# microsoft/tf-gnn-samples

Measured on AMD Instinct MI355X. Metric: edges/sec (whole node), RGCN PPI h=256 training, distinct batches (the reference's epoch-loop definition), higher is better.
Workload: dtype f32; 1 GPU; C2: RGCN on synthetic PPI-shaped batches (~16 graphs, ~1.88 M edges, ~32 k nodes each), 3 edge types [fwd,self,bkwd], h=256, 3 layers, sum aggregation, 1/in-de…; graphs_per_rank=64, max_nodes_in_batch=35964, input_pipeline=ResidentDataset, parallelism=dp1-by-graph

## Files before the change

tf_gnn_samples_amd/_lib.py:

```python
import ctypes
from pathlib import Path

import torch

_PKG_DIR = Path(__file__).resolve().parent
LIB_PATH = _PKG_DIR / "librelgnn.so"

OK, EINVAL, ENOSPC, EHIP, EUNSUPPORTED = 0, 1, 2, 3, 4
ERRFLAG_INDEX_OUT_OF_RANGE = 1
ERRFLAG_NOT_SORTED = 2

AGG_SUM, AGG_MEAN, AGG_SQRT_N, AGG_MAX = 0, 1, 2, 3
MT_MAX = 48
ACT_LINEAR, ACT_TANH, ACT_RELU, ACT_LEAKY_RELU, ACT_ELU, ACT_SELU, ACT_GELU = range(7)

_c_i32, _c_i64, _c_f32 = ctypes.c_int32, ctypes.c_int64, ctypes.c_float
_c_u32 = ctypes.c_uint32
_ptr = ctypes.c_void_p

ABI = {}

ABI["relgnn.h"] = {
    "relgnn_abi_version": (ctypes.c_int, []),
    "relgnn_status_string": (ctypes.c_char_p, [ctypes.c_int]),
# ... 216 lines not shown

ABI["relgnn_sparse_gradient.h"] = {
    "relgnn_named_rows_workspace_bytes": (ctypes.c_size_t, [_c_i64]),
    "relgnn_named_rows_count": (ctypes.c_int, [_ptr, _c_i64, _ptr, _ptr, _ptr, ctypes.c_size_t, _ptr]),
    "relgnn_named_rows_fill": (ctypes.c_int, [_ptr, _c_i64, _ptr, _c_i64, _ptr, _ptr, _ptr, _ptr, _c_i64, _ptr, _ptr, _c_i64, _ptr]),
    "relgnn_rows_l2norm_workspace_bytes": (ctypes.c_size_t, []),
    "relgnn_rows_l2norm": (ctypes.c_int, [_ptr, _c_i64, _ptr, _c_i64, _c_i32, _c_i64, _ptr, _ptr, ctypes.c_size_t, _ptr]),
    "relgnn_rows_adam_step_compact": (ctypes.c_int, [_ptr, _c_i64, _c_i64, _ptr, _ptr, _c_i64, _ptr, _ptr, _c_i64, _c_i32, _ptr, _ptr, _c_i32,
                                                     _c_i32, _ptr, _c_f32, _c_f32, _c_f32, _c_f32, _c_f32, _ptr]),
}

ABI["relgnn_subgraph.h"] = {
    "relgnn_subgraph_supported": (ctypes.c_int, [_c_i64, _c_i32, _c_i64, _c_i32]),
    "relgnn_subgraph_max_walk_length": (_c_i64, []),
    "relgnn_subgraph_workspace_bytes": (ctypes.c_size_t, [_c_i64]),
    "relgnn_subgraph_walk": (ctypes.c_int, [_ptr, _ptr, _c_i64, _c_i32, _ptr, _c_i64, _c_i32, _c_u32, _c_u32, _c_u32, _ptr, _ptr]),
    "relgnn_subgraph_number": (ctypes.c_int, [_ptr, _ptr, _c_i64, _ptr, _c_i64, _ptr]),
    "relgnn_subgraph_induced_count": (ctypes.c_int, [_ptr, _ptr, _c_i64, _c_i32, _ptr, _ptr, _c_i64, _ptr, _ptr, _ptr, _ptr, _ptr,
                                                     ctypes.c_size_t, _ptr]),
    "relgnn_subgraph_induced_emit": (ctypes.c_int, [_ptr, _ptr, _c_i64, _c_i32, _ptr, _c_i64, _c_i64, _ptr, _ptr, _c_i64, _ptr, _ptr,
                                                    _ptr]),
    "relgnn_subgraph_clear": (ctypes.c_int, [_ptr, _c_i64, _ptr, _c_i64, _ptr]),
}

ABI["relgnn_subgraph_norm.h"] = {
    "relgnn_subgraph_visit_count": (ctypes.c_int, [_ptr, _ptr, _c_i64, _c_i32, _c_i64, _ptr, _ptr, _c_i64, _ptr, _ptr, _ptr, _ptr]),
    "relgnn_subgraph_induced_emit_weighted": (ctypes.c_int, [_ptr, _ptr, _c_i64, _c_i32, _c_i64, _ptr, _c_i64, _c_i64, _ptr, _ptr, _ptr,
                                                             _ptr, _c_f32, _c_i64, _ptr, _ptr, _ptr, _ptr]),
    "relgnn_softmax_ce_weighted_stats_workspace_bytes": (ctypes.c_size_t, []),
    "relgnn_softmax_ce_weighted_stats": (ctypes.c_int, [_ptr, _c_i64, _ptr, _ptr, _ptr, _c_f32, _c_i64, _c_i32, _ptr, _ptr,
                                                        ctypes.c_size_t, _ptr]),
    "relgnn_softmax_ce_weighted_bwd": (ctypes.c_int, [_ptr, _c_i64, _ptr, _ptr, _ptr, _c_f32, _c_i64, _c_i32, _ptr, _ptr, _ptr, _c_i64,
                                                      _ptr]),
}

INTERNAL = {}

INTERNAL["graph_partition.h"] = {
    "relgnn_partition_supported": (ctypes.c_int, [_c_i64, _c_i32, _c_i64, _c_i32, _c_i32]),
    "relgnn_partition_wave_row_max": (_c_i64, []),
    "relgnn_partition_wish": (ctypes.c_int, [_ptr, _ptr, _c_i64, _c_i32, _c_i64, _ptr, _ptr, _c_i32, _ptr, _c_i32, _c_u32, _c_u32, _ptr, _ptr,
                                             _c_i64, _c_i32, _ptr, _ptr]),
}

INTERNAL["level_plan.h"] = {
    "relgnn_level_plan_max_levels": (_c_i32, []),
    "relgnn_level_plan_desc_stride": (_c_i64, [_c_i32]),
    "relgnn_level_plan_tile": (_c_i64, []),
    "relgnn_level_plan_workspace_bytes": (ctypes.c_size_t, [_c_i64, _c_i32]),
    "relgnn_level_plan": (ctypes.c_int, [_ptr, _ptr, _ptr, _ptr, _ptr, _ptr, _ptr, _ptr, _ptr, _c_i64, _c_i32, _c_i64, _ptr, _c_i32, _c_i64,
                                         _c_i64, _ptr, _c_i64, _ptr, ctypes.c_size_t, _ptr]),
}

_lib = None


class RelGnnLibraryError(RuntimeError):
    pass


def load_library():
    global _lib
    if _lib is not None:
        return _lib
    if not LIB_PATH.exists():
        raise RelGnnLibraryError(
            "%s not found: the HIP extension is not built. Run `python -c 'import __graft_entry__ as g; "
            "g.build()'` (needs hipcc). There is no CPU fallback for this path." % LIB_PATH)
    lib = ctypes.CDLL(str(LIB_PATH))
    typed = signatures()
    for header, table in INTERNAL.items():
        for name in table:
            if name in typed:
                raise RelGnnLibraryError("%s of csrc/%s is bound twice" % (name, header))
        typed.update(table)
    for name, (restype, argtypes) in typed.items():
        fn = getattr(lib, name)
        fn.restype = restype
        fn.argtypes = argtypes
    if lib.relgnn_abi_version() != 1:
        raise RelGnnLibraryError("librelgnn.so ABI version mismatch")
    _lib = lib
    return lib


def signatures(header=None):
    if header is not None:
        return dict(ABI[header])
    union, owner = {}, {}
    for h, table in ABI.items():
        for name in table:
            if name in owner:
                raise RelGnnLibraryError("%s is bound by both %s and %s" % (name, owner[name], h))
            owner[name] = h
        union.update(table)
    return union


def status_string(code: int) -> str:
    return load_library().relgnn_status_string(code).decode()


def check(code: int, what: str):
    if code == OK:
        return
    msg = "%s failed: %s (status %d)" % (what, status_string(code), code)
# ... 34 lines not shown
```

tf_gnn_samples_amd/csrc/plan_resident.hip:

```cpp
#include "common.h"

using namespace relgnn;

namespace {

__device__ __forceinline__ int upper_slot(const int64_t* __restrict__ table, int n, int64_t x) {
  int lo = 0, hi = n;
  while (hi - lo > 1) {
    const int mid = (lo + hi) >> 1;
    if (table[mid] <= x) lo = mid; else hi = mid;
  }
  return lo;
}

struct BatchTables {
  const int64_t* ids;
  const int64_t* node_off_b;
  const int64_t* msg_off_b;
  const int64_t* edge_off_b;
  const int64_t* type_off_b;
  const int64_t* node_off_d;
  const int64_t* msg_off_d;
  const int64_t* edge_off_d;
  const int64_t* type_off_d;
  int32_t K, L;
  int64_t G;
};

__device__ __forceinline__ int32_t translate_message(const BatchTables& t, int32_t m_d, int l, int k, int64_t g) {
  const int64_t e = (int64_t)m_d - t.type_off_d[l] - t.edge_off_d[(int64_t)l * (t.G + 1) + g];
  return (int32_t)(t.type_off_b[l] + t.edge_off_b[(int64_t)l * (t.K + 1) + k] + e);
}

template <bool FULL>
__global__ __launch_bounds__(256) void assemble_by_target_kernel(
    BatchTables t, int64_t M, const int32_t* __restrict__ perm_d, const int32_t* __restrict__ col_d,
    int32_t* __restrict__ perm_b, int32_t* __restrict__ col_b, int32_t* __restrict__ inv_b,
    const float* __restrict__ w_t_d, int32_t* __restrict__ src_b, float* __restrict__ w_t_b) {
  __shared__ int first_slot;
  for (int64_t base = (int64_t)blockIdx.x * 1024; base < M; base += (int64_t)gridDim.x * 1024) {
    if (threadIdx.x == 0) first_slot = upper_slot(t.msg_off_b, t.K, base);
    __syncthreads();
    int k = first_slot;
    int64_t g = t.ids[k], slot_end = t.msg_off_b[k + 1];
    int64_t msg_delta = t.msg_off_d[g] - t.msg_off_b[k], node_delta = t.node_off_b[k] - t.node_off_d[g];
#pragma unroll
    for (int e = 0; e < 4; ++e) {
      const int64_t p = base + threadIdx.x + 256 * e;
      if (p >= M) break;
      if (p >= slot_end) {
        do { ++k; } while (p >= t.msg_off_b[k + 1]);
        g = t.ids[k]; slot_end = t.msg_off_b[k + 1];
        msg_delta = t.msg_off_d[g] - t.msg_off_b[k]; node_delta = t.node_off_b[k] - t.node_off_d[g];
      }
      const int64_t pd = p + msg_delta;
      const uint32_t c = (uint32_t)col_d[pd];
      const uint32_t cn = c / (uint32_t)t.L;
      const int64_t src = (int64_t)cn + node_delta;
      if (src_b) src_b[p] = (int32_t)src;
      if (w_t_b) w_t_b[p] = w_t_d[pd];
      if constexpr (FULL) {
        const int l = (int)(c - cn * (uint32_t)t.L);
        col_b[p] = (int32_t)(src * t.L + l);
        const int32_t mb = translate_message(t, perm_d[pd], l, k, g);
        perm_b[p] = mb;
        inv_b[mb] = (int32_t)p;
      }
    }
    __syncthreads();
  }
}

template <bool FULL>
__global__ __launch_bounds__(256) void assemble_by_source_kernel(
    BatchTables t, int64_t M, const int32_t* __restrict__ perm_d, const int32_t* __restrict__ frow_d,
    const int32_t* __restrict__ pos_d, int32_t* __restrict__ perm_b, int32_t* __restrict__ frow_b,
    int32_t* __restrict__ tgt_b, int32_t* __restrict__ pos_b, const float* __restrict__ w_s_d, float* __restrict__ w_s_b) {
  __shared__ int first_slot;
  for (int64_t base = (int64_t)blockIdx.x * 1024; base < M; base += (int64_t)gridDim.x * 1024) {
    if (threadIdx.x == 0) first_slot = upper_slot(t.msg_off_b, t.K, base);
    __syncthreads();
    int k = first_slot;
    int64_t g = t.ids[k], slot_end = t.msg_off_b[k + 1];
    int64_t msg_delta = t.msg_off_d[g] - t.msg_off_b[k], node_delta = t.node_off_b[k] - t.node_off_d[g];
#pragma unroll
    for (int e = 0; e < 4; ++e) {
      const int64_t q = base + threadIdx.x + 256 * e;
      if (q >= M) break;
      if (q >= slot_end) {
        do { ++k; } while (q >= t.msg_off_b[k + 1]);
        g = t.ids[k]; slot_end = t.msg_off_b[k + 1];
        msg_delta = t.msg_off_d[g] - t.msg_off_b[k]; node_delta = t.node_off_b[k] - t.node_off_d[g];
      }
      const int64_t qd = q + msg_delta;
      const uint32_t f = (uint32_t)frow_d[qd];
      const uint32_t fn = f / (uint32_t)t.L;
      const int64_t tgt = (int64_t)fn + node_delta;
      tgt_b[q] = (int32_t)tgt;
      if (w_s_b) w_s_b[q] = w_s_d[qd];
      if constexpr (FULL) {
        const int l = (int)(f - fn * (uint32_t)t.L);
        frow_b[q] = (int32_t)(tgt * t.L + l);
        perm_b[q] = translate_message(t, perm_d[qd], l, k, g);
        pos_b[q] = (int32_t)((int64_t)pos_d[qd] - msg_delta);
      }
    }
    __syncthreads();
  }
}

__global__ __launch_bounds__(256) void assemble_rowptr_kernel(
    BatchTables t, int64_t num_buckets, int64_t M, const int32_t* __restrict__ rowptr_t_d,
    const int32_t* __restrict__ rowptr_s_d, int32_t* __restrict__ rowptr_t_b, int32_t* __restrict__ rowptr_s_b) {
  for (int64_t b = blockIdx.x * (int64_t)blockDim.x + threadIdx.x; b <= num_buckets; b += (int64_t)gridDim.x * blockDim.x) {
    if (b == num_buckets) {
      rowptr_t_b[b] = (int32_t)M;
      rowptr_s_b[b] = (int32_t)M;
      continue;
    }
    const int64_t v = b / t.L;
    const int l = (int)(b - v * t.L);
    const int k = upper_slot(t.node_off_b, t.K, v);
    const int64_t g = t.ids[k];
    const int64_t bd = (v - t.node_off_b[k] + t.node_off_d[g]) * t.L + l;
    const int64_t shift = t.msg_off_b[k] - t.msg_off_d[g];
    rowptr_t_b[b] = (int32_t)((int64_t)rowptr_t_d[bd] + shift);
    rowptr_s_b[b] = (int32_t)((int64_t)rowptr_s_d[bd] + shift);
  }
}


__global__ __launch_bounds__(256) void gather_node_rows_kernel(BatchTables t, int64_t V, int32_t cols,
                                                               const uint32_t* __restrict__ src, uint32_t* __restrict__ dst) {
  __shared__ int first_slot;
  const int64_t total = V * cols;
  for (int64_t base = (int64_t)blockIdx.x * 1024; base < total; base += (int64_t)gridDim.x * 1024) {
    if (threadIdx.x == 0) {
      int lo = 0, hi = t.K;
      while (hi - lo > 1) {
        const int mid = (lo + hi) >> 1;
        if (t.node_off_b[mid] * cols <= base) lo = mid; else hi = mid;
      }
      first_slot = lo;
    }
    __syncthreads();
    int k = first_slot;
    int64_t slot_end = t.node_off_b[k + 1] * cols;
    int64_t delta = (t.node_off_d[t.ids[k]] - t.node_off_b[k]) * cols;
#pragma unroll
    for (int e = 0; e < 4; ++e) {
      const int64_t i = base + threadIdx.x + 256 * e;
      if (i < total) {
        if (i >= slot_end) {
          do { ++k; } while (i >= t.node_off_b[k + 1] * cols);
          slot_end = t.node_off_b[k + 1] * cols;
          delta = (t.node_off_d[t.ids[k]] - t.node_off_b[k]) * cols;
        }
        dst[i] = src[delta + i];
      }
    }
    __syncthreads();
  }
}

__global__ __launch_bounds__(256) void gather_degree_kernel(BatchTables t, int64_t V, int64_t N, const float* __restrict__ deg_d,
                                                            float* __restrict__ deg_b, int32_t* __restrict__ node_to_graph) {
  for (int64_t v = blockIdx.x * (int64_t)blockDim.x + threadIdx.x; v < V; v += (int64_t)gridDim.x * blockDim.x) {
    const int k = upper_slot(t.node_off_b, t.K, v);
    const int64_t vd = v - t.node_off_b[k] + t.node_off_d[t.ids[k]];
    for (int l = 0; l < t.L; ++l) deg_b[(int64_t)l * V + v] = deg_d[(int64_t)l * N + vd];
    node_to_graph[v] = k;
  }
}

__global__ __launch_bounds__(256) void gather_adjacency_kernel(BatchTables t, int64_t M, const int2* __restrict__ adj_d,
                                                               int2* __restrict__ adj_b) {
  for (int64_t p = blockIdx.x * (int64_t)blockDim.x + threadIdx.x; p < M; p += (int64_t)gridDim.x * blockDim.x) {
    const int l = upper_slot(t.type_off_b, t.L, p);
    const int64_t e = p - t.type_off_b[l];
    const int64_t* eob = t.edge_off_b + (int64_t)l * (t.K + 1);
    const int k = upper_slot(eob, t.K, e);
    const int64_t g = t.ids[k];
    const int64_t pd = t.type_off_d[l] + t.edge_off_d[(int64_t)l * (t.G + 1) + g] + (e - eob[k]);
    int2 a = adj_d[pd];
    const int off = (int)t.node_off_b[k];
    a.x += off; a.y += off;
    adj_b[p] = a;
  }
}

}

extern "C" {

int relgnn_batch_gather(const int64_t* ids, int32_t num_batch_graphs, int32_t num_edge_types, int64_t num_dataset_graphs,
                        const int64_t* node_off_b, const int64_t* edge_off_b, const int64_t* type_off_b,
                        const int64_t* node_off_d, const int64_t* edge_off_d, const int64_t* type_off_d, int64_t num_nodes,
                        int64_t num_messages, int64_t num_dataset_nodes, int32_t n_payloads, const void* const* h_payload_d,
                        const int32_t* h_payload_cols, void* const* h_payload_b, const float* deg_d, float* deg_b,
                        const int32_t* adj_d, int32_t* adj_b, int32_t* node_to_graph, void* stream) {
  if (num_batch_graphs < 0 || num_edge_types <= 0 || num_dataset_graphs < 0 || num_nodes < 0 || num_messages < 0 ||
      n_payloads < 0 || num_dataset_nodes < 0)
    return RELGNN_EINVAL;
  if (num_batch_graphs == 0 || num_nodes == 0) return RELGNN_OK;
  if (!ids || !node_off_b || !edge_off_b || !type_off_b || !node_off_d || !edge_off_d || !type_off_d) return RELGNN_EINVAL;
  if (n_payloads > 0 && (!h_payload_d || !h_payload_cols || !h_payload_b)) return RELGNN_EINVAL;
  hipStream_t st = as_stream(stream);
  BatchTables t{ids, node_off_b, nullptr, edge_off_b, type_off_b, node_off_d, nullptr, edge_off_d, type_off_d,
                num_batch_graphs, num_edge_types, num_dataset_graphs};
  for (int p = 0; p < n_payloads; ++p) {
    if (h_payload_cols[p] <= 0) continue;
    if (!h_payload_d[p] || !h_payload_b[p]) return RELGNN_EINVAL;
    gather_node_rows_kernel<<<flat_grid((num_nodes * h_payload_cols[p] + 3) / 4, 256), 256, 0, st>>>(
        t, num_nodes, h_payload_cols[p], (const uint32_t*)h_payload_d[p], (uint32_t*)h_payload_b[p]);
  }
  if (deg_b || node_to_graph) {
    if (!deg_d || !deg_b || !node_to_graph) return RELGNN_EINVAL;
    gather_degree_kernel<<<flat_grid(num_nodes, 256), 256, 0, st>>>(t, num_nodes, num_dataset_nodes, deg_d, deg_b, node_to_graph);
  }
  if (num_messages > 0 && adj_b) {
    if (!adj_d) return RELGNN_EINVAL;
    gather_adjacency_kernel<<<flat_grid(num_messages, 256), 256, 0, st>>>(t, num_messages, (const int2*)adj_d, (int2*)adj_b);
  }
  return launch_status();
}

int relgnn_plan_assemble(const int64_t* ids, int32_t num_batch_graphs, int32_t num_edge_types, int64_t num_dataset_graphs,
                         const int64_t* node_off_b, const int64_t* msg_off_b, const int64_t* edge_off_b,
                         const int64_t* type_off_b, const int64_t* node_off_d, const int64_t* msg_off_d,
                         const int64_t* edge_off_d, const int64_t* type_off_d, int64_t num_nodes, int64_t num_messages,
                         const int32_t* rowptr_t_d, const int32_t* perm_t_d, const int32_t* col_t_d,
                         const int32_t* rowptr_s_d, const int32_t* perm_s_d, const int32_t* frow_s_d,
                         const int32_t* pos_t_of_s_d, int32_t* rowptr_t, int32_t* perm_t, int32_t* col_t,
                         int32_t* inv_perm_t, int32_t* rowptr_s, int32_t* perm_s, int32_t* frow_s, int32_t* tgt_s,
                         int32_t* pos_t_of_s, const float* w_t_d, const float* w_s_d, int32_t* src_t, float* w_t, float* w_s,
                         void* stream) {
  if (num_batch_graphs < 0 || num_edge_types <= 0 || num_dataset_graphs < 0 || num_nodes < 0 || num_messages < 0)
    return RELGNN_EINVAL;
  const int64_t buckets = num_nodes * num_edge_types;
  if (buckets >= INT32_MAX || num_messages >= INT32_MAX) return RELGNN_EUNSUPPORTED;
  if (!rowptr_t || !rowptr_s) return RELGNN_EINVAL;
  hipStream_t st = as_stream(stream);
  if (num_batch_graphs == 0 || num_nodes == 0) {
    if (hipMemsetAsync(rowptr_t, 0, (size_t)(buckets + 1) * 4, st) != hipSuccess) return RELGNN_EHIP;
    if (hipMemsetAsync(rowptr_s, 0, (size_t)(buckets + 1) * 4, st) != hipSuccess) return RELGNN_EHIP;
    return RELGNN_OK;
  }
  if (!ids || !node_off_b || !msg_off_b || !edge_off_b || !type_off_b || !node_off_d || !msg_off_d || !edge_off_d ||
      !type_off_d || !rowptr_t_d || !rowptr_s_d)
    return RELGNN_EINVAL;
  BatchTables t{ids, node_off_b, msg_off_b, edge_off_b, type_off_b, node_off_d, msg_off_d, edge_off_d, type_off_d,
                num_batch_graphs, num_edge_types, num_dataset_graphs};
  assemble_rowptr_kernel<<<flat_grid(buckets + 1, 256), 256, 0, st>>>(t, buckets, num_messages, rowptr_t_d, rowptr_s_d,
                                                                      rowptr_t, rowptr_s);
  if (num_messages > 0) {
    const bool full = perm_t || col_t || inv_perm_t || perm_s || frow_s || pos_t_of_s;
    if (full && (!perm_t || !col_t || !inv_perm_t || !perm_s || !frow_s || !pos_t_of_s || !perm_t_d || !perm_s_d || !pos_t_of_s_d))
      return RELGNN_EINVAL;
    if (!col_t_d || !frow_s_d || !tgt_s) return RELGNN_EINVAL;
    if (!full && !src_t) return RELGNN_EINVAL;
    if ((w_t && !w_t_d) || (w_s && !w_s_d)) return RELGNN_EINVAL;
    const dim3 grid = flat_grid((num_messages + 3) / 4, 256);
    if (full) {
      assemble_by_target_kernel<true><<<grid, 256, 0, st>>>(t, num_messages, perm_t_d, col_t_d, perm_t, col_t, inv_perm_t,
                                                            w_t_d, src_t, w_t);
      assemble_by_source_kernel<true><<<grid, 256, 0, st>>>(t, num_messages, perm_s_d, frow_s_d, pos_t_of_s_d, perm_s, frow_s,
                                                            tgt_s, pos_t_of_s, w_s_d, w_s);
    } else {
      assemble_by_target_kernel<false><<<grid, 256, 0, st>>>(t, num_messages, nullptr, col_t_d, nullptr, nullptr, nullptr,
                                                             w_t_d, src_t, w_t);
      assemble_by_source_kernel<false><<<grid, 256, 0, st>>>(t, num_messages, nullptr, frow_s_d, nullptr, nullptr, nullptr,
                                                             tgt_s, nullptr, w_s_d, w_s);
    }
  }
  return launch_status();
}

}
```

tf_gnn_samples_amd/tasks/resident.py:

```python
from typing import Iterator, Optional, Sequence

import numpy as np
import torch

from .. import _lib
from .. import config as _cfg
from ..graph import RelGraph
from .batcher import GraphStore
from .sparse_graph_task import DeviceBatch


def _dev_i64(a, device):
    return torch.as_tensor(np.ascontiguousarray(a, dtype=np.int64), device=device)


class ResidentDataset:
    def __init__(self, store: GraphStore, device, features: str = "initial_node_features",
                 constants: Optional[dict] = None):
        self.store, self.device = store, torch.device(device)
        if self.device.type != "cuda":
            raise _lib.RelGnnLibraryError("a resident data fold lives in HBM; got device %s" % self.device)
        self.features, self.constants = features, dict(constants or {})
        G, L = store.num_graphs, store.num_edge_types
        dev = self.device
        self.node_off = store.node_off
        self.edge_off = np.stack(store.edge_off) if L else np.zeros((0, G + 1), np.int64)
        per_graph_msgs = (self.edge_off[:, 1:] - self.edge_off[:, :-1]).sum(0) if L else np.zeros(G, np.int64)
        self.msg_off = np.concatenate([[0], np.cumsum(per_graph_msgs)]).astype(np.int64)
        self.type_off = np.concatenate([[0], np.cumsum(self.edge_off[:, -1])]).astype(np.int64)
        N, M = int(self.node_off[-1]), int(self.msg_off[-1])
        if N * max(L, 1) >= 2 ** 31 - 1 or M >= 2 ** 31 - 1:
            raise ValueError("data fold too large for one int32-indexed union; use the host batcher")
        self.payload_d = [torch.as_tensor(a, device=dev) for a in store.payload]
        self.graph_payload_d = {k: torch.as_tensor(v, device=dev) for k, v in store.graph_payload.items()}
        self.deg_d = torch.stack([torch.as_tensor(a, device=dev) for a in store.deg]) if L else torch.zeros((0, N), device=dev)
        self.adj_d = [torch.as_tensor(a, device=dev) for a in store.adj]
        self.node_off_d, self.msg_off_d = _dev_i64(self.node_off, dev), _dev_i64(self.msg_off, dev)
        self.edge_off_d, self.type_off_d = _dev_i64(self.edge_off, dev), _dev_i64(self.type_off, dev)
        union = []
        for l in range(L):
            counts = torch.as_tensor(self.edge_off[l, 1:] - self.edge_off[l, :-1], device=dev)
            shift = torch.repeat_interleave(self.node_off_d[:-1], counts).to(torch.int32)
            union.append((self.adj_d[l] + shift.unsqueeze(1)).contiguous())
        g = RelGraph(union, N, validate=True)
        self._has_hubs = g.has_long_buckets
        self.pair_counts = None
        if L >= 8:
            cnt = np.zeros((2, G, L), dtype=np.int64)
            for l in range(L):
                a = np.asarray(store.adj[l]).reshape(-1, 2)
                gidx = np.repeat(np.arange(G), np.diff(self.edge_off[l]))
                for side in (0, 1):
                    key = gidx.astype(np.int64) * (N + 1) + a[:, 1 - side].astype(np.int64) + self.node_off[gidx]
                    cnt[side, :, l] = np.bincount(np.unique(key) // (N + 1), minlength=G)
            self.pair_counts = cnt
        self.plan_d = dict(rowptr_t=g.rowptr_t, perm_t=g.perm_t, col_t=g.col_t, rowptr_s=g.rowptr_s, perm_s=g.perm_s,
                           frow_s=g.frow_s, pos_t_of_s=g.pos_t_of_s)
        self.w_t_d = g.degree_scale(self.deg_d) if M > 0 else torch.zeros(0, device=dev)
        self.w_s_d = g.w_by_source(self.w_t_d) if M > 0 else torch.zeros(0, device=dev)
        self.adj_flat_d = torch.cat(self.adj_d).contiguous() if L else torch.zeros((0, 2), dtype=torch.int32, device=dev)
        self._fast = [i for i, t in enumerate(self.payload_d) if t.element_size() == 4 and t.is_contiguous()]
        self._fast_cols = [int(self.payload_d[i][0].numel()) if self.payload_d[i].shape[0] else 1 for i in self._fast]
        self._num_nodes_fold = N
        self._stage = [None] * 4
        self._stage_done = [None] * 4
        self._stage_at = 0

    def _staging(self, n: int) -> torch.Tensor:
        k = self._stage_at
        self._stage_at = (k + 1) % len(self._stage)
        if self._stage_done[k] is not None:
            self._stage_done[k].synchronize()
        buf = self._stage[k]
        if buf is None or buf.numel() < n:
            buf = torch.empty(max(n, 1024) * 2, dtype=torch.int64).pin_memory()
            self._stage[k] = buf
        return buf, k

    def assemble(self, graph_ids: Sequence[int], lean: bool = True) -> DeviceBatch:
        import ctypes
        dev, L, G = self.device, self.store.num_edge_types, self.store.num_graphs
        ids = np.ascontiguousarray(np.asarray(graph_ids, dtype=np.int64))
        K = len(ids)
        nodes = self.node_off[ids + 1] - self.node_off[ids]
        edges = self.edge_off[:, ids + 1] - self.edge_off[:, ids]
        node_off_b = np.concatenate([[0], np.cumsum(nodes)])
        edge_off_b = np.concatenate([np.zeros((L, 1), np.int64), np.cumsum(edges, axis=1)], axis=1)
        msg_off_b = np.concatenate([[0], np.cumsum(edges.sum(0))])
        type_off_b = np.concatenate([[0], np.cumsum(edge_off_b[:, -1])])
        V, M = int(node_off_b[-1]), int(msg_off_b[-1])
        sizes = [K, K + 1, K + 1, L + 1, L * (K + 1)]
        total = sum(sizes)
        host, slot = self._staging(total)
        hn = host.numpy()
        at = 0
        for part in (ids, node_off_b, msg_off_b, type_off_b, edge_off_b.reshape(-1)):
            hn[at:at + part.size] = part
            at += part.size
        tab = host[:total].to(dev, non_blocking=True)
        ev = torch.cuda.Event()
        ev.record(torch.cuda.current_stream(dev))
        self._stage_done[slot] = ev
        o = np.cumsum([0] + sizes)
        ids_d, node_off_bd, msg_off_bd, type_off_bd, edge_off_bd = (tab[o[i]:o[i + 1]] for i in range(5))
        type_off = [int(x) for x in type_off_b]
        i32 = lambda n: torch.empty(int(n), dtype=torch.int32, device=dev)

        names = self.store.payload_names
        payload = {}
        out_fast = []
        for i in self._fast:
            src = self.payload_d[i]
            out_fast.append(torch.empty((V,) + tuple(src.shape[1:]), dtype=src.dtype, device=dev))
            payload[names[i]] = out_fast[-1]
        deg = torch.empty((L, V), dtype=torch.float32, device=dev)
        n2g = torch.empty(V, dtype=torch.int32, device=dev)
        nf = len(self._fast)
        arr = ctypes.c_void_p * max(nf, 1)

        def gather(n_payloads, with_node_tables, adj_flat):
            _lib.launch("relgnn_batch_gather", _lib.ptr(ids_d), K, L, G, _lib.ptr(node_off_bd), _lib.ptr(edge_off_bd),
                        _lib.ptr(type_off_bd), _lib.ptr(self.node_off_d), _lib.ptr(self.edge_off_d), _lib.ptr(self.type_off_d), V, M,
                        self._num_nodes_fold, n_payloads, arr(*[self.payload_d[i].data_ptr() for i in self._fast]),
                        (ctypes.c_int32 * max(nf, 1))(*self._fast_cols), arr(*[t.data_ptr() for t in out_fast]), _lib.ptr(self.deg_d),
                        _lib.ptr(deg) if with_node_tables else None, _lib.ptr(self.adj_flat_d), _lib.ptr(adj_flat),
                        _lib.ptr(n2g) if with_node_tables else None)

        def split_types(adj_flat):
            return [adj_flat[type_off[l]:type_off[l + 1]] for l in range(L)]

        adj_flat = None if lean else torch.empty((M, 2), dtype=torch.int32, device=dev)
        gather(nf, True, adj_flat)
        if len(self._fast) < len(names):
            node_idx = (torch.arange(V, device=dev) - node_off_bd[n2g.long()] + self.node_off_d[ids_d[n2g.long()]])
            for i, name in enumerate(names):
                if i not in self._fast:
                    payload[name] = self.payload_d[i].index_select(0, node_idx)
        for name, flat in self.graph_payload_d.items():
            payload[name] = flat.index_select(0, ids_d)

        S = V * L
        rowptr_t, rowptr_s, tgt_s, src_t = i32(S + 1), i32(S + 1), i32(M), i32(M)
        w_t = torch.empty(M, dtype=torch.float32, device=dev)
        w_s = torch.empty(M, dtype=torch.float32, device=dev)
        d = self.plan_d

        def plan(full):
            six = {k: (i32(M) if full else None) for k in RelGraph._LAZY_ARRAYS}
            _lib.launch("relgnn_plan_assemble", _lib.ptr(ids_d), K, L, G, _lib.ptr(node_off_bd), _lib.ptr(msg_off_bd),
                        _lib.ptr(edge_off_bd), _lib.ptr(type_off_bd), _lib.ptr(self.node_off_d), _lib.ptr(self.msg_off_d),
                        _lib.ptr(self.edge_off_d), _lib.ptr(self.type_off_d), V, M, _lib.ptr(d["rowptr_t"]), _lib.ptr(d["perm_t"]),
                        _lib.ptr(d["col_t"]), _lib.ptr(d["rowptr_s"]), _lib.ptr(d["perm_s"]), _lib.ptr(d["frow_s"]),
                        _lib.ptr(d["pos_t_of_s"]), _lib.ptr(rowptr_t), _lib.ptr(six["perm_t"]), _lib.ptr(six["col_t"]),
                        _lib.ptr(six["inv_perm_t"]), _lib.ptr(rowptr_s), _lib.ptr(six["perm_s"]), _lib.ptr(six["frow_s"]), _lib.ptr(tgt_s),
                        _lib.ptr(six["pos_t_of_s"]), _lib.ptr(self.w_t_d), _lib.ptr(self.w_s_d), _lib.ptr(src_t), _lib.ptr(w_t),
                        _lib.ptr(w_s))
            return six

        state = {"adj": None if lean else split_types(adj_flat)}

        def adjacency():
            if state["adj"] is None:
                tab.record_stream(torch.cuda.current_stream(dev))
                flat = torch.empty((M, 2), dtype=torch.int32, device=dev)
                gather(0, False, flat)
                state["adj"] = split_types(flat)
            return state["adj"]

        def complete():
            tab.record_stream(torch.cuda.current_stream(dev))
            return {"adjacency_lists": adjacency(), **plan(True)}

        six = plan(not lean)
        if lean:
            graph = RelGraph.from_arrays(None, V, rowptr_t=rowptr_t, rowptr_s=rowptr_s, tgt_s=tgt_s,
                                         edge_counts=[type_off[l + 1] - type_off[l] for l in range(L)], complete=complete)
        else:
            graph = RelGraph.from_arrays(state["adj"], V, rowptr_t=rowptr_t, rowptr_s=rowptr_s, tgt_s=tgt_s, **six)
        graph.preset_degree_scale(deg, src_t, w_t, w_s)
        if self.pair_counts is not None:
            graph.pair_counts = (self.pair_counts[0, ids].sum(0).tolist(), self.pair_counts[1, ids].sum(0).tolist())
        if self._has_hubs:
            graph.split_long_segments()
        batch = DeviceBatch.from_tensors(
            num_graphs=K, num_nodes=V, num_edges=M, initial_node_features=payload[self.features],
            adjacency_lists=adjacency if lean else state["adj"],
            type_to_num_incoming_edges=deg, graph_nodes_list=n2g,
            extra={**{k: v for k, v in payload.items() if k != self.features}, **self.constants})
        batch.graph = graph
        return batch

    def iterate(self, graph_ids: Sequence[int], max_nodes_per_batch: int) -> Iterator[DeviceBatch]:
        for ids in self.store.split_batches(graph_ids, max_nodes_per_batch):
            yield self.assemble(ids)
```

Measured before the change: 1.056 billion edges/sec.

## Fuse lean batch assembly into one multi-job kernel with a single arena allocation

The default lean path now runs payload gathers, degree gather, rowptr assembly and the by-target/by-source edge assembly as block ranges of one kernel launch, instead of several separate launches. All outputs are carved from one device arena rather than many torch.empty calls, which cuts host-side launch and allocator overhead per batch. The assembly loops are also restructured to issue all four gathered loads before any stores, for more memory-level parallelism. The cost is a more complex dispatch kernel and a payload cap of eight per launch, with more handled by extra launches.

```diff
diff --git a/tf_gnn_samples_amd/_lib.py b/tf_gnn_samples_amd/_lib.py
--- a/tf_gnn_samples_amd/_lib.py
+++ b/tf_gnn_samples_amd/_lib.py
@@ -292,6 +292,11 @@
                                          _c_i64, _ptr, _c_i64, _ptr, ctypes.c_size_t, _ptr]),
 }
 
+INTERNAL["plan_resident.h"] = {
+    "relgnn_batch_assemble_lean": (ctypes.c_int, [_ptr, _c_i32, _c_i32, _c_i64] + [_ptr] * 4 + [_c_i64, _c_i64, _c_i64, _c_i32] + [_ptr] * 3
+                                   + [_ptr] * 3 + [_ptr] * 6 + [_ptr] * 6 + [_ptr]),
+}
+
 _lib = None
 
 
diff --git a/tf_gnn_samples_amd/csrc/plan_resident.h b/tf_gnn_samples_amd/csrc/plan_resident.h
--- /dev/null
+++ b/tf_gnn_samples_amd/csrc/plan_resident.h
@@ -0,0 +1,23 @@
+#ifndef RELGNN_PLAN_RESIDENT_H_
+#define RELGNN_PLAN_RESIDENT_H_
+
+#include <stdint.h>
+
+#ifdef __cplusplus
+extern "C" {
+#endif
+
+int relgnn_batch_assemble_lean(const int64_t* ids, int32_t num_batch_graphs, int32_t num_edge_types, int64_t num_dataset_graphs,
+                               const int64_t* node_off_b, const int64_t* msg_off_b, const int64_t* node_off_d,
+                               const int64_t* msg_off_d, int64_t num_nodes, int64_t num_messages, int64_t num_dataset_nodes,
+                               int32_t n_payloads, const void* const* h_payload_d, const int32_t* h_payload_cols,
+                               void* const* h_payload_b, const float* deg_d, float* deg_b, int32_t* node_to_graph,
+                               const int32_t* rowptr_t_d, const int32_t* col_t_d, const int32_t* rowptr_s_d,
+                               const int32_t* frow_s_d, const float* w_t_d, const float* w_s_d, int32_t* rowptr_t,
+                               int32_t* rowptr_s, int32_t* src_t, int32_t* tgt_s, float* w_t, float* w_s, void* stream);
+
+#ifdef __cplusplus
+}
+#endif
+
+#endif
diff --git a/tf_gnn_samples_amd/csrc/plan_resident.hip b/tf_gnn_samples_amd/csrc/plan_resident.hip
--- a/tf_gnn_samples_amd/csrc/plan_resident.hip
+++ b/tf_gnn_samples_amd/csrc/plan_resident.hip
@@ -1,4 +1,5 @@
 #include "common.h"
+#include "plan_resident.h"
 
 using namespace relgnn;
 
@@ -33,38 +34,122 @@
 }
 
 template <bool FULL>
+__device__ __forceinline__ void assemble_by_target_body(
+    unsigned block, unsigned nblocks, int* first_slot, const BatchTables& t, int64_t M, const int32_t* __restrict__ perm_d,
+    const int32_t* __restrict__ col_d, int32_t* __restrict__ perm_b, int32_t* __restrict__ col_b, int32_t* __restrict__ inv_b,
+    const float* __restrict__ w_t_d, int32_t* __restrict__ src_b, float* __restrict__ w_t_b) {
+  for (int64_t base = (int64_t)block * 1024; base < M; base += (int64_t)nblocks * 1024) {
+    if (threadIdx.x == 0) *first_slot = upper_slot(t.msg_off_b, t.K, base);
+    __syncthreads();
+    int k = *first_slot;
+    int64_t g = t.ids[k], slot_end = t.msg_off_b[k + 1];
+    int64_t msg_delta = t.msg_off_d[g] - t.msg_off_b[k], node_delta = t.node_off_b[k] - t.node_off_d[g];
+    int64_t pd[4], nd[4], gs[4];
+    int ks[4];
+#pragma unroll
+    for (int e = 0; e < 4; ++e) {
+      const int64_t p = base + threadIdx.x + 256 * e;
+      if (p < M) {
+        if (p >= slot_end) {
+          do { ++k; } while (p >= t.msg_off_b[k + 1]);
+          g = t.ids[k]; slot_end = t.msg_off_b[k + 1];
+          msg_delta = t.msg_off_d[g] - t.msg_off_b[k]; node_delta = t.node_off_b[k] - t.node_off_d[g];
+        }
+        pd[e] = p + msg_delta; nd[e] = node_delta; ks[e] = k; gs[e] = g;
+      }
+    }
+    uint32_t c[4];
+    float w[4];
+    int32_t m_d[4];
+#pragma unroll
+    for (int e = 0; e < 4; ++e) {
+      if (base + threadIdx.x + 256 * e < M) {
+        c[e] = (uint32_t)col_d[pd[e]];
+        if (w_t_b) w[e] = w_t_d[pd[e]];
+        if constexpr (FULL) m_d[e] = perm_d[pd[e]];
+      }
+    }
+#pragma unroll
+    for (int e = 0; e < 4; ++e) {
+      const int64_t p = base + threadIdx.x + 256 * e;
+      if (p < M) {
+        const uint32_t cn = c[e] / (uint32_t)t.L;
+        const int64_t src = (int64_t)cn + nd[e];
+        if (src_b) src_b[p] = (int32_t)src;
+        if (w_t_b) w_t_b[p] = w[e];
+        if constexpr (FULL) {
+          const int l = (int)(c[e] - cn * (uint32_t)t.L);
+          col_b[p] = (int32_t)(src * t.L + l);
+          const int32_t mb = translate_message(t, m_d[e], l, ks[e], gs[e]);
+          perm_b[p] = mb;
+          inv_b[mb] = (int32_t)p;
+        }
+      }
+    }
+    __syncthreads();
+  }
+}
+
+template <bool FULL>
 __global__ __launch_bounds__(256) void assemble_by_target_kernel(
     BatchTables t, int64_t M, const int32_t* __restrict__ perm_d, const int32_t* __restrict__ col_d,
     int32_t* __restrict__ perm_b, int32_t* __restrict__ col_b, int32_t* __restrict__ inv_b,
     const float* __restrict__ w_t_d, int32_t* __restrict__ src_b, float* __restrict__ w_t_b) {
   __shared__ int first_slot;
-  for (int64_t base = (int64_t)blockIdx.x * 1024; base < M; base += (int64_t)gridDim.x * 1024) {
-    if (threadIdx.x == 0) first_slot = upper_slot(t.msg_off_b, t.K, base);
-    __syncthreads();
-    int k = first_slot;
+  assemble_by_target_body<FULL>(blockIdx.x, gridDim.x, &first_slot, t, M, perm_d, col_d, perm_b, col_b, inv_b, w_t_d, src_b, w_t_b);
+}
+
+template <bool FULL>
+__device__ __forceinline__ void assemble_by_source_body(
+    unsigned block, unsigned nblocks, int* first_slot, const BatchTables& t, int64_t M, const int32_t* __restrict__ perm_d,
+    const int32_t* __restrict__ frow_d, const int32_t* __restrict__ pos_d, int32_t* __restrict__ perm_b,
+    int32_t* __restrict__ frow_b, int32_t* __restrict__ tgt_b, int32_t* __restrict__ pos_b, const float* __restrict__ w_s_d,
+    float* __restrict__ w_s_b) {
+  for (int64_t base = (int64_t)block * 1024; base < M; base += (int64_t)nblocks * 1024) {
+    if (threadIdx.x == 0) *first_slot = upper_slot(t.msg_off_b, t.K, base);
+    __syncthreads();
+    int k = *first_slot;
     int64_t g = t.ids[k], slot_end = t.msg_off_b[k + 1];
     int64_t msg_delta = t.msg_off_d[g] - t.msg_off_b[k], node_delta = t.node_off_b[k] - t.node_off_d[g];
-#pragma unroll
-    for (int e = 0; e < 4; ++e) {
-      const int64_t p = base + threadIdx.x + 256 * e;
-      if (p >= M) break;
-      if (p >= slot_end) {
-        do { ++k; } while (p >= t.msg_off_b[k + 1]);
-        g = t.ids[k]; slot_end = t.msg_off_b[k + 1];
-        msg_delta = t.msg_off_d[g] - t.msg_off_b[k]; node_delta = t.node_off_b[k] - t.node_off_d[g];
-      }
-      const int64_t pd = p + msg_delta;
-      const uint32_t c = (uint32_t)col_d[pd];
-      const uint32_t cn = c / (uint32_t)t.L;
-      const int64_t src = (int64_t)cn + node_delta;
-      if (src_b) src_b[p] = (int32_t)src;
-      if (w_t_b) w_t_b[p] = w_t_d[pd];
-      if constexpr (FULL) {
-        const int l = (int)(c - cn * (uint32_t)t.L);
-        col_b[p] = (int32_t)(src * t.L + l);
-        const int32_t mb = translate_message(t, perm_d[pd], l, k, g);
-        perm_b[p] = mb;
-        inv_b[mb] = (int32_t)p;
+    int64_t qd[4], nd[4], md[4], gs[4];
+    int ks[4];
+#pragma unroll
+    for (int e = 0; e < 4; ++e) {
+      const int64_t q = base + threadIdx.x + 256 * e;
+      if (q < M) {
+        if (q >= slot_end) {
+          do { ++k; } while (q >= t.msg_off_b[k + 1]);
+          g = t.ids[k]; slot_end = t.msg_off_b[k + 1];
+          msg_delta = t.msg_off_d[g] - t.msg_off_b[k]; node_delta = t.node_off_b[k] - t.node_off_d[g];
+        }
+        qd[e] = q + msg_delta; nd[e] = node_delta; md[e] = msg_delta; ks[e] = k; gs[e] = g;
+      }
+    }
+    uint32_t f[4];
+    float w[4];
+    int32_t m_d[4], pos[4];
+#pragma unroll
+    for (int e = 0; e < 4; ++e) {
+      if (base + threadIdx.x + 256 * e < M) {
+        f[e] = (uint32_t)frow_d[qd[e]];
+        if (w_s_b) w[e] = w_s_d[qd[e]];
+        if constexpr (FULL) { m_d[e] = perm_d[qd[e]]; pos[e] = pos_d[qd[e]]; }
+      }
+    }
+#pragma unroll
+    for (int e = 0; e < 4; ++e) {
+      const int64_t q = base + threadIdx.x + 256 * e;
+      if (q < M) {
+        const uint32_t fn = f[e] / (uint32_t)t.L;
+        const int64_t tgt = (int64_t)fn + nd[e];
+        tgt_b[q] = (int32_t)tgt;
+        if (w_s_b) w_s_b[q] = w[e];
+        if constexpr (FULL) {
+          const int l = (int)(f[e] - fn * (uint32_t)t.L);
+          frow_b[q] = (int32_t)(tgt * t.L + l);
+          perm_b[q] = translate_message(t, m_d[e], l, ks[e], gs[e]);
+          pos_b[q] = (int32_t)((int64_t)pos[e] - md[e]);
+        }
       }
     }
     __syncthreads();
@@ -77,42 +162,15 @@
     const int32_t* __restrict__ pos_d, int32_t* __restrict__ perm_b, int32_t* __restrict__ frow_b,
     int32_t* __restrict__ tgt_b, int32_t* __restrict__ pos_b, const float* __restrict__ w_s_d, float* __restrict__ w_s_b) {
   __shared__ int first_slot;
-  for (int64_t base = (int64_t)blockIdx.x * 1024; base < M; base += (int64_t)gridDim.x * 1024) {
-    if (threadIdx.x == 0) first_slot = upper_slot(t.msg_off_b, t.K, base);
-    __syncthreads();
-    int k = first_slot;
-    int64_t g = t.ids[k], slot_end = t.msg_off_b[k + 1];
-    int64_t msg_delta = t.msg_off_d[g] - t.msg_off_b[k], node_delta = t.node_off_b[k] - t.node_off_d[g];
-#pragma unroll
-    for (int e = 0; e < 4; ++e) {
-      const int64_t q = base + threadIdx.x + 256 * e;
-      if (q >= M) break;
-      if (q >= slot_end) {
-        do { ++k; } while (q >= t.msg_off_b[k + 1]);
-        g = t.ids[k]; slot_end = t.msg_off_b[k + 1];
-        msg_delta = t.msg_off_d[g] - t.msg_off_b[k]; node_delta = t.node_off_b[k] - t.node_off_d[g];
-      }
-      const int64_t qd = q + msg_delta;
-      const uint32_t f = (uint32_t)frow_d[qd];
-      const uint32_t fn = f / (uint32_t)t.L;
-      const int64_t tgt = (int64_t)fn + node_delta;
-      tgt_b[q] = (int32_t)tgt;
-      if (w_s_b) w_s_b[q] = w_s_d[qd];
-      if constexpr (FULL) {
-        const int l = (int)(f - fn * (uint32_t)t.L);
-        frow_b[q] = (int32_t)(tgt * t.L + l);
-        perm_b[q] = translate_message(t, perm_d[qd], l, k, g);
-        pos_b[q] = (int32_t)((int64_t)pos_d[qd] - msg_delta);
-      }
-    }
-    __syncthreads();
-  }
-}
-
-__global__ __launch_bounds__(256) void assemble_rowptr_kernel(
-    BatchTables t, int64_t num_buckets, int64_t M, const int32_t* __restrict__ rowptr_t_d,
-    const int32_t* __restrict__ rowptr_s_d, int32_t* __restrict__ rowptr_t_b, int32_t* __restrict__ rowptr_s_b) {
-  for (int64_t b = blockIdx.x * (int64_t)blockDim.x + threadIdx.x; b <= num_buckets; b += (int64_t)gridDim.x * blockDim.x) {
+  assemble_by_source_body<FULL>(blockIdx.x, gridDim.x, &first_slot, t, M, perm_d, frow_d, pos_d, perm_b, frow_b, tgt_b, pos_b,
+                                w_s_d, w_s_b);
+}
+
+__device__ __forceinline__ void assemble_rowptr_body(
+    unsigned block, unsigned nblocks, const BatchTables& t, int64_t num_buckets, int64_t M,
+    const int32_t* __restrict__ rowptr_t_d, const int32_t* __restrict__ rowptr_s_d, int32_t* __restrict__ rowptr_t_b,
+    int32_t* __restrict__ rowptr_s_b) {
+  for (int64_t b = block * (int64_t)blockDim.x + threadIdx.x; b <= num_buckets; b += (int64_t)nblocks * blockDim.x) {
     if (b == num_buckets) {
       rowptr_t_b[b] = (int32_t)M;
       rowptr_s_b[b] = (int32_t)M;
@@ -129,24 +187,31 @@
   }
 }
 
-
-__global__ __launch_bounds__(256) void gather_node_rows_kernel(BatchTables t, int64_t V, int32_t cols,
-                                                               const uint32_t* __restrict__ src, uint32_t* __restrict__ dst) {
-  __shared__ int first_slot;
+__global__ __launch_bounds__(256) void assemble_rowptr_kernel(
+    BatchTables t, int64_t num_buckets, int64_t M, const int32_t* __restrict__ rowptr_t_d,
+    const int32_t* __restrict__ rowptr_s_d, int32_t* __restrict__ rowptr_t_b, int32_t* __restrict__ rowptr_s_b) {
+  assemble_rowptr_body(blockIdx.x, gridDim.x, t, num_buckets, M, rowptr_t_d, rowptr_s_d, rowptr_t_b, rowptr_s_b);
+}
+
+
+__device__ __forceinline__ void gather_node_rows_body(unsigned block, unsigned nblocks, int* first_slot, const BatchTables& t,
+                                                      int64_t V, int32_t cols, const uint32_t* __restrict__ src,
+                                                      uint32_t* __restrict__ dst) {
   const int64_t total = V * cols;
-  for (int64_t base = (int64_t)blockIdx.x * 1024; base < total; base += (int64_t)gridDim.x * 1024) {
+  for (int64_t base = (int64_t)block * 1024; base < total; base += (int64_t)nblocks * 1024) {
     if (threadIdx.x == 0) {
       int lo = 0, hi = t.K;
       while (hi - lo > 1) {
         const int mid = (lo + hi) >> 1;
         if (t.node_off_b[mid] * cols <= base) lo = mid; else hi = mid;
       }
-      first_slot = lo;
-    }
-    __syncthreads();
-    int k = first_slot;
+      *first_slot = lo;
+    }
+    __syncthreads();
+    int k = *first_slot;
     int64_t slot_end = t.node_off_b[k + 1] * cols;
     int64_t delta = (t.node_off_d[t.ids[k]] - t.node_off_b[k]) * cols;
+    int64_t from[4];
 #pragma unroll
     for (int e = 0; e < 4; ++e) {
       const int64_t i = base + threadIdx.x + 256 * e;
@@ -156,21 +221,42 @@
           slot_end = t.node_off_b[k + 1] * cols;
           delta = (t.node_off_d[t.ids[k]] - t.node_off_b[k]) * cols;
         }
-        dst[i] = src[delta + i];
-      }
-    }
-    __syncthreads();
-  }
-}
-
-__global__ __launch_bounds__(256) void gather_degree_kernel(BatchTables t, int64_t V, int64_t N, const float* __restrict__ deg_d,
-                                                            float* __restrict__ deg_b, int32_t* __restrict__ node_to_graph) {
-  for (int64_t v = blockIdx.x * (int64_t)blockDim.x + threadIdx.x; v < V; v += (int64_t)gridDim.x * blockDim.x) {
+        from[e] = delta + i;
+      }
+    }
+    uint32_t x[4];
+#pragma unroll
+    for (int e = 0; e < 4; ++e)
+      if (base + threadIdx.x + 256 * e < total) x[e] = src[from[e]];
+#pragma unroll
+    for (int e = 0; e < 4; ++e) {
+      const int64_t i = base + threadIdx.x + 256 * e;
+      if (i < total) dst[i] = x[e];
+    }
+    __syncthreads();
+  }
+}
+
+__global__ __launch_bounds__(256) void gather_node_rows_kernel(BatchTables t, int64_t V, int32_t cols,
+                                                               const uint32_t* __restrict__ src, uint32_t* __restrict__ dst) {
+  __shared__ int first_slot;
+  gather_node_rows_body(blockIdx.x, gridDim.x, &first_slot, t, V, cols, src, dst);
+}
+
+__device__ __forceinline__ void gather_degree_body(unsigned block, unsigned nblocks, const BatchTables& t, int64_t V, int64_t N,
+                                                   const float* __restrict__ deg_d, float* __restrict__ deg_b,
+                                                   int32_t* __restrict__ node_to_graph) {
+  for (int64_t v = block * (int64_t)blockDim.x + threadIdx.x; v < V; v += (int64_t)nblocks * blockDim.x) {
     const int k = upper_slot(t.node_off_b, t.K, v);
     const int64_t vd = v - t.node_off_b[k] + t.node_off_d[t.ids[k]];
     for (int l = 0; l < t.L; ++l) deg_b[(int64_t)l * V + v] = deg_d[(int64_t)l * N + vd];
     node_to_graph[v] = k;
   }
+}
+
+__global__ __launch_bounds__(256) void gather_degree_kernel(BatchTables t, int64_t V, int64_t N, const float* __restrict__ deg_d,
+                                                            float* __restrict__ deg_b, int32_t* __restrict__ node_to_graph) {
+  gather_degree_body(blockIdx.x, gridDim.x, t, V, N, deg_d, deg_b, node_to_graph);
 }
 
 __global__ __launch_bounds__(256) void gather_adjacency_kernel(BatchTables t, int64_t M, const int2* __restrict__ adj_d,
@@ -186,6 +272,44 @@
     const int off = (int)t.node_off_b[k];
     a.x += off; a.y += off;
     adj_b[p] = a;
+  }
+}
+
+constexpr int LEAN_MAX_PAYLOADS = 8;
+constexpr int LEAN_FIXED_JOBS = 4;
+
+struct LeanBatch {
+  BatchTables t;
+  int64_t V, M, N;
+  int32_t n_payloads;
+  uint32_t end[LEAN_MAX_PAYLOADS + LEAN_FIXED_JOBS];
+  int32_t payload_cols[LEAN_MAX_PAYLOADS];
+  const uint32_t* payload_d[LEAN_MAX_PAYLOADS];
+  uint32_t* payload_b[LEAN_MAX_PAYLOADS];
+  const float* deg_d; float* deg_b; int32_t* node_to_graph;
+  const int32_t* rowptr_t_d; const int32_t* rowptr_s_d; int32_t* rowptr_t_b; int32_t* rowptr_s_b;
+  const int32_t* col_t_d; const float* w_t_d; int32_t* src_t_b; float* w_t_b;
+  const int32_t* frow_s_d; const float* w_s_d; int32_t* tgt_s_b; float* w_s_b;
+};
+
+__global__ __launch_bounds__(256) void batch_assemble_lean_kernel(LeanBatch a) {
+  __shared__ int first_slot;
+  const int last = a.n_payloads + LEAN_FIXED_JOBS - 1;
+  int j = 0;
+  while (j < last && blockIdx.x >= a.end[j]) ++j;
+  const unsigned first = j ? a.end[j - 1] : 0u;
+  const unsigned block = blockIdx.x - first, nblocks = a.end[j] - first;
+  if (j < a.n_payloads) {
+    gather_node_rows_body(block, nblocks, &first_slot, a.t, a.V, a.payload_cols[j], a.payload_d[j], a.payload_b[j]);
+    return;
+  }
+  switch (j - a.n_payloads) {
+    case 0: gather_degree_body(block, nblocks, a.t, a.V, a.N, a.deg_d, a.deg_b, a.node_to_graph); break;
+    case 1: assemble_rowptr_body(block, nblocks, a.t, a.V * a.t.L, a.M, a.rowptr_t_d, a.rowptr_s_d, a.rowptr_t_b, a.rowptr_s_b); break;
+    case 2: assemble_by_target_body<false>(block, nblocks, &first_slot, a.t, a.M, nullptr, a.col_t_d, nullptr, nullptr, nullptr,
+                                           a.w_t_d, a.src_t_b, a.w_t_b); break;
+    default: assemble_by_source_body<false>(block, nblocks, &first_slot, a.t, a.M, nullptr, a.frow_s_d, nullptr, nullptr, nullptr,
+                                            a.tgt_s_b, nullptr, a.w_s_d, a.w_s_b); break;
   }
 }
 
@@ -276,4 +400,58 @@
   return launch_status();
 }
 
-}
+int relgnn_batch_assemble_lean(const int64_t* ids, int32_t num_batch_graphs, int32_t num_edge_types, int64_t num_dataset_graphs,
+                               const int64_t* node_off_b, const int64_t* msg_off_b, const int64_t* node_off_d,
+                               const int64_t* msg_off_d, int64_t num_nodes, int64_t num_messages, int64_t num_dataset_nodes,
+                               int32_t n_payloads, const void* const* h_payload_d, const int32_t* h_payload_cols,
+                               void* const* h_payload_b, const float* deg_d, float* deg_b, int32_t* node_to_graph,
+                               const int32_t* rowptr_t_d, const int32_t* col_t_d, const int32_t* rowptr_s_d,
+                               const int32_t* frow_s_d, const float* w_t_d, const float* w_s_d, int32_t* rowptr_t,
+                               int32_t* rowptr_s, int32_t* src_t, int32_t* tgt_s, float* w_t, float* w_s, void* stream) {
+  if (num_batch_graphs < 0 || num_edge_types <= 0 || num_dataset_graphs < 0 || num_nodes < 0 || num_messages < 0 ||
+      n_payloads < 0 || num_dataset_nodes < 0)
+    return RELGNN_EINVAL;
+  const int64_t V = num_batch_graphs == 0 ? 0 : num_nodes, M = V == 0 ? 0 : num_messages;
+  const int64_t buckets = V * num_edge_types;
+  if (buckets >= INT32_MAX || M >= INT32_MAX) return RELGNN_EUNSUPPORTED;
+  if (!rowptr_t || !rowptr_s) return RELGNN_EINVAL;
+  if (V > 0 && (!ids || !node_off_b || !msg_off_b || !node_off_d || !msg_off_d || !rowptr_t_d || !rowptr_s_d)) return RELGNN_EINVAL;
+  if (V > 0 && (!deg_d || !deg_b || !node_to_graph)) return RELGNN_EINVAL;
+  if (V > 0 && n_payloads > 0 && (!h_payload_d || !h_payload_cols || !h_payload_b)) return RELGNN_EINVAL;
+  if (M > 0 && (!col_t_d || !frow_s_d || !src_t || !tgt_s || (w_t && !w_t_d) || (w_s && !w_s_d))) return RELGNN_EINVAL;
+  hipStream_t st = as_stream(stream);
+  LeanBatch a{};
+  a.t = BatchTables{ids, node_off_b, msg_off_b, nullptr, nullptr, node_off_d, msg_off_d, nullptr, nullptr,
+                    num_batch_graphs, num_edge_types, num_dataset_graphs};
+  a.V = V; a.M = M; a.N = num_dataset_nodes;
+  a.deg_d = deg_d; a.deg_b = deg_b; a.node_to_graph = node_to_graph;
+  a.rowptr_t_d = rowptr_t_d; a.rowptr_s_d = rowptr_s_d; a.rowptr_t_b = rowptr_t; a.rowptr_s_b = rowptr_s;
+  a.col_t_d = col_t_d; a.w_t_d = w_t_d; a.src_t_b = src_t; a.w_t_b = w_t;
+  a.frow_s_d = frow_s_d; a.w_s_d = w_s_d; a.tgt_s_b = tgt_s; a.w_s_b = w_s;
+  const int32_t P = V > 0 ? n_payloads : 0;
+  for (int32_t p0 = 0; p0 == 0 || p0 < P; p0 += LEAN_MAX_PAYLOADS) {
+    a.n_payloads = P - p0 < LEAN_MAX_PAYLOADS ? P - p0 : LEAN_MAX_PAYLOADS;
+    unsigned end = 0;
+    for (int32_t p = 0; p < a.n_payloads; ++p) {
+      const int32_t cols = h_payload_cols[p0 + p];
+      if (cols > 0) {
+        if (!h_payload_d[p0 + p] || !h_payload_b[p0 + p]) return RELGNN_EINVAL;
+        end += flat_grid((V * cols + 3) / 4, 256);
+      }
+      a.payload_cols[p] = cols;
+      a.payload_d[p] = (const uint32_t*)h_payload_d[p0 + p];
+      a.payload_b[p] = (uint32_t*)h_payload_b[p0 + p];
+      a.end[p] = end;
+    }
+    const bool rest = p0 == 0;
+    uint32_t* fixed = a.end + a.n_payloads;
+    fixed[0] = end += rest && V > 0 ? flat_grid(V, 256) : 0;
+    fixed[1] = end += rest ? flat_grid(buckets + 1, 256) : 0;
+    fixed[2] = end += rest && M > 0 ? flat_grid((M + 3) / 4, 256) : 0;
+    fixed[3] = end += rest && M > 0 ? flat_grid((M + 3) / 4, 256) : 0;
+    if (end > 0) batch_assemble_lean_kernel<<<end, 256, 0, st>>>(a);
+  }
+  return launch_status();
+}
+
+}
diff --git a/tf_gnn_samples_amd/tasks/resident.py b/tf_gnn_samples_amd/tasks/resident.py
--- a/tf_gnn_samples_amd/tasks/resident.py
+++ b/tf_gnn_samples_amd/tasks/resident.py
@@ -1,3 +1,4 @@
+import ctypes
 from typing import Iterator, Optional, Sequence
 
 import numpy as np
@@ -62,6 +63,14 @@
         self._fast = [i for i, t in enumerate(self.payload_d) if t.element_size() == 4 and t.is_contiguous()]
         self._fast_cols = [int(self.payload_d[i][0].numel()) if self.payload_d[i].shape[0] else 1 for i in self._fast]
         self._num_nodes_fold = N
+        nf = max(len(self._fast), 1)
+        self._lean_payload_d = (ctypes.c_void_p * nf)(*[_lib.ptr(self.payload_d[i]) for i in self._fast])
+        self._lean_payload_cols = (ctypes.c_int32 * nf)(*self._fast_cols)
+        self._lean_payload_b = (ctypes.c_void_p * nf)()
+        self._lean_offsets_d = (_lib.ptr(self.node_off_d), _lib.ptr(self.msg_off_d))
+        self._lean_deg_d = _lib.ptr(self.deg_d)
+        self._lean_fold_d = (_lib.ptr(self.plan_d["rowptr_t"]), _lib.ptr(self.plan_d["col_t"]), _lib.ptr(self.plan_d["rowptr_s"]),
+                             _lib.ptr(self.plan_d["frow_s"]), _lib.ptr(self.w_t_d), _lib.ptr(self.w_s_d))
         self._stage = [None] * 4
         self._stage_done = [None] * 4
         self._stage_at = 0
@@ -77,8 +86,40 @@
             self._stage[k] = buf
         return buf, k
 
+    def _assemble_lean(self, tab: torch.Tensor, table_at, K: int, V: int, M: int):
+        L, S = self.store.num_edge_types, V * self.store.num_edge_types
+        words = [V * c for c in self._fast_cols] + [L * V, V, S + 1, S + 1, M, M, M, M]
+        at, total = [], 0
+        for n in words:
+            at.append(total)
+            total += (n + 3) & ~3
+        arena = torch.empty(total * 4, dtype=torch.uint8, device=self.device)
+        typed = {}
+
+        def view(j, dtype, shape=None):
+            base = typed.get(dtype)
+            if base is None:
+                base = typed[dtype] = arena.view(dtype)
+            v = base[at[j]:at[j] + words[j]]
+            return v if shape is None else v.view(shape)
+
+        nf = len(self._fast)
+        out_fast = [view(j, self.payload_d[i].dtype, (V,) + tuple(self.payload_d[i].shape[1:])) for j, i in enumerate(self._fast)]
+        deg, n2g = view(nf, torch.float32, (L, V)), view(nf + 1, torch.int32)
+        rowptr_t, rowptr_s, src_t, tgt_s = (view(nf + j, torch.int32) for j in (2, 3, 4, 5))
+        w_t, w_s = view(nf + 6, torch.float32), view(nf + 7, torch.float32)
+        a0, t0 = arena.data_ptr(), tab.data_ptr()
+        out = [a0 + 4 * x for x in at]
+        for j in range(nf):
+            self._lean_payload_b[j] = out[j]
+        ids_p, node_off_p, msg_off_p = (t0 + 8 * int(table_at[j]) for j in range(3))
+        _lib.launch("relgnn_batch_assemble_lean", ids_p, K, L, self.store.num_graphs, node_off_p, msg_off_p, *self._lean_offsets_d,
+                    V, M, self._num_nodes_fold, nf, self._lean_payload_d, self._lean_payload_cols, self._lean_payload_b,
+                    self._lean_deg_d, out[nf], out[nf + 1], *self._lean_fold_d, out[nf + 2], out[nf + 3], out[nf + 4],
+                    out[nf + 5], out[nf + 6], out[nf + 7])
+        return out_fast, deg, n2g, rowptr_t, rowptr_s, src_t, tgt_s, w_t, w_s
+
     def assemble(self, graph_ids: Sequence[int], lean: bool = True) -> DeviceBatch:
-        import ctypes
         dev, L, G = self.device, self.store.num_edge_types, self.store.num_graphs
         ids = np.ascontiguousarray(np.asarray(graph_ids, dtype=np.int64))
         K = len(ids)
@@ -107,14 +148,18 @@
         i32 = lambda n: torch.empty(int(n), dtype=torch.int32, device=dev)
 
         names = self.store.payload_names
-        payload = {}
-        out_fast = []
-        for i in self._fast:
-            src = self.payload_d[i]
-            out_fast.append(torch.empty((V,) + tuple(src.shape[1:]), dtype=src.dtype, device=dev))
-            payload[names[i]] = out_fast[-1]
-        deg = torch.empty((L, V), dtype=torch.float32, device=dev)
-        n2g = torch.empty(V, dtype=torch.int32, device=dev)
+        S = V * L
+        if lean:
+            out_fast, deg, n2g, rowptr_t, rowptr_s, src_t, tgt_s, w_t, w_s = self._assemble_lean(tab, o, K, V, M)
+        else:
+            out_fast = [torch.empty((V,) + tuple(self.payload_d[i].shape[1:]), dtype=self.payload_d[i].dtype, device=dev)
+                        for i in self._fast]
+            deg = torch.empty((L, V), dtype=torch.float32, device=dev)
+            n2g = torch.empty(V, dtype=torch.int32, device=dev)
+            rowptr_t, rowptr_s, tgt_s, src_t = i32(S + 1), i32(S + 1), i32(M), i32(M)
+            w_t = torch.empty(M, dtype=torch.float32, device=dev)
+            w_s = torch.empty(M, dtype=torch.float32, device=dev)
+        payload = {names[i]: t for i, t in zip(self._fast, out_fast)}
         nf = len(self._fast)
         arr = ctypes.c_void_p * max(nf, 1)
 
@@ -130,7 +175,8 @@
             return [adj_flat[type_off[l]:type_off[l + 1]] for l in range(L)]
 
         adj_flat = None if lean else torch.empty((M, 2), dtype=torch.int32, device=dev)
-        gather(nf, True, adj_flat)
+        if not lean:
+            gather(nf, True, adj_flat)
         if len(self._fast) < len(names):
             node_idx = (torch.arange(V, device=dev) - node_off_bd[n2g.long()] + self.node_off_d[ids_d[n2g.long()]])
             for i, name in enumerate(names):
@@ -139,14 +185,10 @@
         for name, flat in self.graph_payload_d.items():
             payload[name] = flat.index_select(0, ids_d)
 
-        S = V * L
-        rowptr_t, rowptr_s, tgt_s, src_t = i32(S + 1), i32(S + 1), i32(M), i32(M)
-        w_t = torch.empty(M, dtype=torch.float32, device=dev)
-        w_s = torch.empty(M, dtype=torch.float32, device=dev)
         d = self.plan_d
 
-        def plan(full):
-            six = {k: (i32(M) if full else None) for k in RelGraph._LAZY_ARRAYS}
+        def plan():
+            six = {k: i32(M) for k in RelGraph._LAZY_ARRAYS}
             _lib.launch("relgnn_plan_assemble", _lib.ptr(ids_d), K, L, G, _lib.ptr(node_off_bd), _lib.ptr(msg_off_bd),
                         _lib.ptr(edge_off_bd), _lib.ptr(type_off_bd), _lib.ptr(self.node_off_d), _lib.ptr(self.msg_off_d),
                         _lib.ptr(self.edge_off_d), _lib.ptr(self.type_off_d), V, M, _lib.ptr(d["rowptr_t"]), _lib.ptr(d["perm_t"]),
@@ -169,14 +211,13 @@
 
         def complete():
             tab.record_stream(torch.cuda.current_stream(dev))
-            return {"adjacency_lists": adjacency(), **plan(True)}
-
-        six = plan(not lean)
+            return {"adjacency_lists": adjacency(), **plan()}
+
         if lean:
             graph = RelGraph.from_arrays(None, V, rowptr_t=rowptr_t, rowptr_s=rowptr_s, tgt_s=tgt_s,
                                          edge_counts=[type_off[l + 1] - type_off[l] for l in range(L)], complete=complete)
         else:
-            graph = RelGraph.from_arrays(state["adj"], V, rowptr_t=rowptr_t, rowptr_s=rowptr_s, tgt_s=tgt_s, **six)
+            graph = RelGraph.from_arrays(state["adj"], V, rowptr_t=rowptr_t, rowptr_s=rowptr_s, tgt_s=tgt_s, **plan())
         graph.preset_degree_scale(deg, src_t, w_t, w_s)
         if self.pair_counts is not None:
             graph.pair_counts = (self.pair_counts[0, ids].sum(0).tolist(), self.pair_counts[1, ids].sum(0).tolist())
```

Result: faster. 1.072 billion edges/sec, median of 5 (+1.5%).
